# HiLab-git/FPL-plus

Measured on AMD Instinct MI355X. Metric: 3D volumes/sec (train step, 80x160x160), higher is better.
Workload: dtype bf16; 1 GPU; UNet3D-DSBN 32-base-ch bf16 (fp32 master weights), per-GPU batch 2x1x80x160x160 synthetic VS crops, DiceLoss + Adam, domain alternating per step; global_batch=2, parallelism=dp1, step=zero_grad+forward+loss+backward+allreduce+adam

## Files before the change

fpl-plus_amd/csrc/common.h:

```cpp
#pragma once
#include <hip/hip_runtime.h>
#include <math.h>
#include <stdint.h>
#include <stdio.h>
#include <stdarg.h>
#include <string.h>
#include "../../include/fplx.h"

typedef __bf16 bf16_t;

#define FPLX_WAVE 64

inline char* fplx_err_buf() {
  static thread_local char buf[512];
  return buf;
}
inline int fplx_fail(int code, const char* fmt, ...) {
  va_list ap;
  va_start(ap, fmt);
  vsnprintf(fplx_err_buf(), 512, fmt, ap);
  va_end(ap);
  return code;
}
inline int fplx_check_launch(const char* what) {
  hipError_t e = hipGetLastError();
  if (e != hipSuccess) return fplx_fail(FPLX_E_HIP, "%s: %s", what, hipGetErrorString(e));
  return FPLX_OK;
}
#define FPLX_REQUIRE(cond, code, ...) \
  do {                                 \
    if (!(cond)) return fplx_fail(code, __VA_ARGS__); \
  } while (0)

template <typename T> struct Act;
template <> struct Act<float> {
  static __device__ __forceinline__ float ld(const float* p) { return *p; }
  static __device__ __forceinline__ void st(float* p, float v) { *p = v; }
};
template <> struct Act<bf16_t> {
  static __device__ __forceinline__ float ld(const bf16_t* p) { return (float)*p; }
  static __device__ __forceinline__ void st(bf16_t* p, float v) { *p = (bf16_t)v; }
};

__device__ __forceinline__ float ld_dt(const void* p, int64_t i, int dt) {
  return dt == FPLX_F32 ? ((const float*)p)[i] : (float)((const bf16_t*)p)[i];
}
__device__ __forceinline__ void st_dt(void* p, int64_t i, int dt, float v) {
  if (dt == FPLX_F32) ((float*)p)[i] = v;
  else ((bf16_t*)p)[i] = (bf16_t)v;
}

__device__ __forceinline__ float wave_sum(float v) {
#pragma unroll
  for (int o = 32; o > 0; o >>= 1) v += __shfl_xor(v, o, 64);
  return v;
}
__device__ __forceinline__ double wave_sum_d(double v) {
#pragma unroll
  for (int o = 32; o > 0; o >>= 1) v += __shfl_xor(v, o, 64);
  return v;
}

#ifdef __HIPCC__
struct FplxAdamConst { float step_size, b1, b2, eps, wd, inv_sqrt_bc2, gscale, omb1, omb2; };
__device__ __forceinline__ void fplx_adam_elem(float& pi, float g, float& mi, float& vi, const FplxAdamConst& c) {
  const float gi = fmaf(c.wd, pi, g * c.gscale);
  mi = fmaf(c.b1, mi, c.omb1 * gi);
  vi = fmaf(c.b2, vi, (c.omb2 * gi) * gi);
  const float denom = fmaf(sqrtf(vi), c.inv_sqrt_bc2, c.eps);
  pi = fmaf(-c.step_size, mi / denom, pi);
}
struct FplxOptimConst { float lr, wd, gscale, k0, k1, k2, k3, k4; int first; };
__device__ __forceinline__ float fplx_optim_grad(float pi, float g, const FplxOptimConst& c) {
  return fmaf(c.wd, pi, g * c.gscale);
}
template <bool MOM>
__device__ __forceinline__ void fplx_sgd_elem(float& pi, float g, float& buf, const FplxOptimConst& c) {
  const float gi = fplx_optim_grad(pi, g, c);
  if (MOM) {
    buf = fmaf(c.k0, buf, gi);
    pi = fmaf(-c.lr, buf, pi);
  } else {
    pi = fmaf(-c.lr, gi, pi);
  }
}
__device__ __forceinline__ void fplx_adadelta_elem(float& pi, float g, float& sq, float& acc, const FplxOptimConst& c) {
  const float gi = fplx_optim_grad(pi, g, c);
  sq = fmaf(c.k0, sq, (c.k1 * gi) * gi);
  const float stdv = sqrtf(sq + c.k2);
  const float ratio = sqrtf(acc + c.k2) / stdv;
  const float delta = ratio * gi;
  acc = fmaf(c.k0, acc, (c.k1 * delta) * delta);
  pi = fmaf(-c.lr, delta, pi);
}
__device__ __forceinline__ void fplx_adagrad_elem(float& pi, float g, float& sum, const FplxOptimConst& c) {
  const float gi = fplx_optim_grad(pi, g, c);
  sum = fmaf(gi, gi, sum);
  const float stdv = sqrtf(sum) + c.k2;
  pi = fmaf(-c.lr, gi / stdv, pi);
}
__device__ __forceinline__ void fplx_adamax_elem(float& pi, float g, float& mi, float& ui, const FplxOptimConst& c) {
  const float gi = fplx_optim_grad(pi, g, c);
  mi = fmaf(c.k0, mi, c.k1 * gi);
  const float decayed = c.k3 * ui;
  ui = fmaxf(decayed, fabsf(gi) + c.k2);
  pi = fmaf(-c.lr, mi / ui, pi);
}
__device__ __forceinline__ void fplx_asgd_elem(float& pi, float g, float& ax, const FplxOptimConst& c) {
  const float gi = fplx_optim_grad(pi, g, c);
  const float decayed = pi * c.k0;
  pi = fmaf(-c.lr, gi, decayed);
  const float d = pi - ax;
  ax = c.k3 == 1.f ? pi : fmaf(d, c.k3, ax);
}
template <bool MOM>
__device__ __forceinline__ void fplx_rmsprop_elem(float& pi, float g, float& sq, float& buf, const FplxOptimConst& c) {
  const float gi = fplx_optim_grad(pi, g, c);
  sq = fmaf(c.k0, sq, (c.k1 * gi) * gi);
  const float avg = sqrtf(sq) + c.k2;
  if (MOM) {
    buf = fmaf(c.k3, buf, gi / avg);
    pi = fmaf(-c.lr, buf, pi);
  } else {
    pi = fmaf(-c.lr, gi / avg, pi);
  }
}
__device__ __forceinline__ void fplx_rprop_elem(float& pi, float g, float& prev, float& ss, const FplxOptimConst& c) {
  float gi = g * c.gscale;
  if (c.first) { prev = 0.f; ss = c.lr; }
  const float s = gi * prev;
  const float f = s > 0.f ? c.k1 : (s < 0.f ? c.k0 : 1.f);
  const float scaled = ss * f;
  ss = fminf(fmaxf(scaled, c.k3), c.k4);
  if (s < 0.f) gi = 0.f;
  const float sg = gi > 0.f ? 1.f : (gi < 0.f ? -1.f : 0.f);
  pi = fmaf(-sg, ss, pi);
  prev = gi;
}
template <int KIND, int NS>
__device__ __forceinline__ void fplx_optim_elem(float& pi, float g, float& s0, float& s1, const FplxOptimConst& c) {
  if constexpr (KIND == FPLX_OPT_SGD) fplx_sgd_elem<NS == 1>(pi, g, s0, c);
  else if constexpr (KIND == FPLX_OPT_ADADELTA) fplx_adadelta_elem(pi, g, s0, s1, c);
  else if constexpr (KIND == FPLX_OPT_ADAGRAD) fplx_adagrad_elem(pi, g, s0, c);
  else if constexpr (KIND == FPLX_OPT_ADAMAX) fplx_adamax_elem(pi, g, s0, s1, c);
  else if constexpr (KIND == FPLX_OPT_ASGD) fplx_asgd_elem(pi, g, s0, c);
  else if constexpr (KIND == FPLX_OPT_RMSPROP) fplx_rmsprop_elem<NS == 2>(pi, g, s0, s1, c);
  else fplx_rprop_elem(pi, g, s0, s1, c);
}
#define FPLX_OPTIM_DISPATCH(kind, ns, X)                                       \
  switch ((kind) * 4 + (ns)) {                                                 \
    case FPLX_OPT_SGD * 4 + 0: X(FPLX_OPT_SGD, 0); break;                      \
    case FPLX_OPT_SGD * 4 + 1: X(FPLX_OPT_SGD, 1); break;                      \
    case FPLX_OPT_ADADELTA * 4 + 2: X(FPLX_OPT_ADADELTA, 2); break;            \
    case FPLX_OPT_ADAGRAD * 4 + 1: X(FPLX_OPT_ADAGRAD, 1); break;              \
    case FPLX_OPT_ADAMAX * 4 + 2: X(FPLX_OPT_ADAMAX, 2); break;                \
    case FPLX_OPT_ASGD * 4 + 1: X(FPLX_OPT_ASGD, 1); break;                    \
    case FPLX_OPT_RMSPROP * 4 + 1: X(FPLX_OPT_RMSPROP, 1); break;              \
    case FPLX_OPT_RMSPROP * 4 + 2: X(FPLX_OPT_RMSPROP, 2); break;              \
    default: X(FPLX_OPT_RPROP, 2); break;                                      \
  }
static inline int fplx_optim_consts(const char* who, int kind, const float* hp, int nhp, int step, float gscale, const void* s0,
                                    const void* s1, FplxOptimConst* c, int* ns) {
  static const int want[FPLX_OPT_COUNT] = {3, 4, 4, 5, 4, 5, 5};
  FPLX_REQUIRE(kind >= 0 && kind < FPLX_OPT_COUNT, FPLX_E_BADSHAPE, "%s: unknown optimiser kind %d (0..%d)", who, kind,
               FPLX_OPT_COUNT - 1);
  FPLX_REQUIRE(hp, FPLX_E_NULL, "%s: null hyper-parameter array", who);
  FPLX_REQUIRE(nhp == want[kind], FPLX_E_BADSHAPE, "%s: kind %d takes %d hyper-parameters, got %d", who, kind, want[kind], nhp);
  FPLX_REQUIRE(step >= 1, FPLX_E_BADSHAPE, "%s: step=%d (1-based)", who, step);
  *c = {hp[0], 0.f, gscale, 0.f, 0.f, 0.f, 0.f, 0.f, step == 1};
  int need = 2;
  switch (kind) {
    case FPLX_OPT_SGD:
      c->k0 = hp[1]; c->wd = hp[2];
      need = hp[1] != 0.f ? 1 : 0;
      break;
    case FPLX_OPT_ADADELTA:
      c->k0 = hp[1]; c->k1 = (float)(1.0 - (double)hp[1]); c->k2 = hp[2]; c->wd = hp[3];
      break;
    case FPLX_OPT_ADAGRAD:
      c->lr = (float)((double)hp[0] / (1.0 + (double)(step - 1) * (double)hp[1])); c->k2 = hp[2]; c->wd = hp[3];
      need = 1;
      break;
    case FPLX_OPT_ADAMAX:
      c->lr = (float)((double)hp[0] / (1.0 - pow((double)hp[1], step)));
      c->k0 = hp[1]; c->k1 = (float)(1.0 - (double)hp[1]); c->k3 = hp[2]; c->k2 = hp[3]; c->wd = hp[4];
      break;
    case FPLX_OPT_ASGD:
      c->k0 = (float)(1.0 - (double)hp[2] * (double)hp[0]); c->k3 = hp[1]; c->wd = hp[3];
      need = 1;
      break;
    case FPLX_OPT_RMSPROP:
      c->k0 = hp[1]; c->k1 = (float)(1.0 - (double)hp[1]); c->k2 = hp[2]; c->k3 = hp[3]; c->wd = hp[4];
      need = hp[3] > 0.f ? 2 : 1;
      break;
    default:
      c->k0 = hp[1]; c->k1 = hp[2]; c->k3 = hp[3]; c->k4 = hp[4];
      break;
  }
  FPLX_REQUIRE((need < 1 || s0) && (need < 2 || s1), FPLX_E_NULL, "%s: kind %d needs %d state buffer(s) here", who, kind, need);
  *ns = need;
  return FPLX_OK;
}
struct FplxBlock { int x, y, z; };
__device__ __forceinline__ FplxBlock fplx_xcd_block(int on) {
  FplxBlock b = {(int)blockIdx.x, (int)blockIdx.y, (int)blockIdx.z};
  if (!on) return b;
  const unsigned gx = gridDim.x, gy = gridDim.y, gz = gridDim.z, t = gx * gy * gz;
  const unsigned l = (blockIdx.z * gy + blockIdx.y) * gx + blockIdx.x;
  const unsigned xcd = l & 7u, q = t >> 3, r = t & 7u;
  const unsigned lp = xcd * q + (xcd < r ? xcd : r) + (l >> 3);
  const unsigned per = gy * gz, xq = lp / per, rem = lp - xq * per;
  b.x = __builtin_amdgcn_readfirstlane((int)xq);
  b.z = __builtin_amdgcn_readfirstlane((int)(rem / gy));
  b.y = __builtin_amdgcn_readfirstlane((int)(rem % gy));
  return b;
}
struct FplxTileRange { int64_t first, end, step; };
__device__ __forceinline__ FplxTileRange fplx_xcd_tiles(int64_t ntiles, int on) {
  FplxTileRange t = {(int64_t)blockIdx.x, ntiles, (int64_t)gridDim.x};
  if (!on || gridDim.x < 16) return t;
  const unsigned c = blockIdx.x & 7u, xcd = (blockIdx.y * gridDim.x + blockIdx.x) & 7u;
  const int64_t q = ntiles >> 3, r = ntiles & 7;
  const int64_t start = xcd * q + ((int64_t)xcd < r ? xcd : r);
  t.first = start + (blockIdx.x >> 3);
  t.end = start + q + ((int64_t)xcd < r ? 1 : 0);
  t.step = (gridDim.x - c + 7u) >> 3;
  return t;
}
template <typename... P, typename... A>
inline void fplx_launch(void (*kernel)(P...), dim3 grid, dim3 block, size_t lds, hipStream_t st, A... args) {
  if (lds) (void)hipFuncSetAttribute((const void*)kernel, hipFuncAttributeMaxDynamicSharedMemorySize, (int)lds);
  kernel<<<grid, block, lds, st>>>(args...);
}
#endif
#define FPLX_KNOB_LIST(X)                                                                                              \
  X(XCD, "xcd", 1)                                                    \
  X(BRICK, "brick", 1)                                    \
  X(BRICK_FILL, "brick_fill", 192)           \
  X(BRICK_GEO, "brick_geo", -1)                    \
  X(BRICK_KSPLIT, "brick_ksplit", 0)                                             \
  X(EDGE_BLOCKS, "edge_blocks", 1024)                             \
  X(STEM_ROWS, "stem_rows", 1)                                              \
  X(OUTCONV_T, "outconv_t", 1)                                 \
  X(OUTCONV_DGRAD_MFMA, "outconv_dgrad_mfma", 1)                                                                       \
  X(OUTCONV_FWD_ROWS, "outconv_fwd_rows", 1)  \
  X(OUTCONV_DGRAD_ROWS, "outconv_dgrad_rows", 1)  \
  X(PACK_TILED, "pack_tiled", 1)                                                                                       \
  X(PACK_MULTI, "pack_multi", 1)                                                                                       \
  X(MARCH, "march", 1)                               \
  X(MARCH64_FW, "march64_fw", 0)                                \
  X(MARCH_DS, "march_ds", 0)                                       \
  X(MARCH128, "march128", 1)                                                                                           \
  X(MARCH64_LW, "march64_lw", 1)            \
  X(MARCH32_V2, "march32_v2", 4)              \
  X(WG_COT_MINVOX, "wg_cot_minvox", 0)                                                                                 \
  X(WG_TW, "wg_tw", 0)                                                                                                 \
  X(WG_CIT, "wg_cit", 2)                                                                                               \
  X(WG_COT, "wg_cot", 2)                                                                                               \
  X(WG_DS, "wg_ds", 0)                                                                                                 \
  X(WG_VOX, "wg_vox", 1)                              \
  X(WG_ROLL, "wg_roll", 1)                     \
  X(WG_ROLL_GEO, "wg_roll_geo", 0)          \
  X(WG_ROLL_M16, "wg_roll_m16", 1)                 \
  X(WG_ROLL_MB, "wg_roll_mb", 1)            \
  X(WG_ROLL_CUS, "wg_roll_cus", 256)                                \
  X(WG_ROLL_OVH, "wg_roll_ovh", 9)                     \
  X(WG_ROLL_MINVOX, "wg_roll_minvox", 0)                                                   \
  X(WG_ROLL2D, "wg_roll2d", 1)              \
  X(WG_ROLL2D_OVH, "wg_roll2d_ovh", 3)      \
  X(WG_REDUCE_ROWS, "wg_reduce_rows", 8)    \
  X(WG_VOX_LW, "wg_vox_lw", 1)              \
  X(WG_VOX_CUS, "wg_vox_cus", 128)          \
  X(WG_VOX_MAXV, "wg_vox_maxv", 10000)         \
  X(STREAM_MIN_W, "stream_min_w", 64)                                                                                  \
  X(TILE_MT, "tile_mt", 0)                                                                                             \
  X(TILE_NT, "tile_nt", 0)                                                                                             \
  X(TILE_KS, "tile_ks", 0)                                                                                             \
  X(MID_TILE, "mid_tile", 1)                                                                                           \
  X(DECONV_ROWS, "deconv_rows", 1)                                                                                     \
  X(DECONV_DGRAD_ROWS, "deconv_dgrad_rows", 1)   \
  X(ROWS_SMALL_DIV, "rows_small_div", 16)   \
  X(EW_GROUP, "ew_group", 1)                                                                                           \
  X(POOL_COL, "pool_col", 1)                         \
  X(EW_INFLIGHT, "ew_inflight", 2)          \
  X(EW_INFLIGHT_REDUCE, "ew_inflight_reduce", 2)
enum FplxKnobId {
#define FPLX_KNOB_ENUM(id, key, def) FPLX_K_##id,
  FPLX_KNOB_LIST(FPLX_KNOB_ENUM)
#undef FPLX_KNOB_ENUM
  FPLX_K_COUNT
};
extern "C" __attribute__((visibility("hidden"))) int64_t fplx_knob_values[FPLX_K_COUNT];
static inline int64_t fplx_knob(int id) { return __atomic_load_n(&fplx_knob_values[id], __ATOMIC_RELAXED); }
static inline int fplx_xcd_on() { return (int)fplx_knob(FPLX_K_XCD); }

static inline int fplx_rows_for(int64_t voxels) {
  constexpr int cap = 512;
  const int div = voxels <= 32768 ? (int)fplx_knob(FPLX_K_ROWS_SMALL_DIV) : 64;
  int64_t r = (voxels + div - 1) / div;
  if (r > cap) r = cap;
  if (r < 1) r = 1;
  return (int)r;
}
```

fpl-plus_amd/csrc/conv_mfma.hip:

```cpp
#include "internal.h"
#include "gfx950.h"
#include <stdlib.h>

namespace {

constexpr int DIRECT_THREADS = 256;

template <int MT, int NTL, int MODE>
__global__ void __launch_bounds__(DIRECT_THREADS)
conv_fwd_direct(const bf16_t* __restrict__ x, int64_t ldx, const bf16_t* __restrict__ wp,
                const float* __restrict__ bias, bf16_t* __restrict__ y, int64_t ldy, int N, int D, int H, int W,
                int Cin, int Cout, float* __restrict__ stats, float* __restrict__ partial = nullptr) {
  const int lane = threadIdx.x & 63, wave = threadIdx.x >> 6;
  const int r = lane & 31, kh8 = (lane >> 5) * 8;
  const int64_t V = (int64_t)N * D * H * W;
  const int64_t m0 = ((int64_t)blockIdx.x * 4 + wave) * (MT * 32);
  const int n0 = blockIdx.y * (NTL * 32);

  int vn[MT], vd[MT], vh[MT], vw[MT];
  bool vok[MT];
#pragma unroll
  for (int t = 0; t < MT; ++t) {
    int64_t v = m0 + t * 32 + r;
    vok[t] = v < V;
// ... 1929 lines not shown
  bool fits;
  StreamCfg stream;
  DirectCfg direct;
};

static FwdPlan fwd_plan(int n, int d, int h, int w, int cin, int cout, int mid) {
  FwdPlan p = {};
  p.kernel = FPLX_KERNEL_GENERIC; p.geo = -1; p.ksplit = 1; p.tap_cnt = 27;
  if (cin % 16 != 0 || cout % 32 != 0) return p;
  const int64_t V = (int64_t)n * d * h * w;
  p.fits = V < ((int64_t)1 << 31);
  auto split = [&](int rows) {
    p.stats_rows = p.ksplit > 1 ? splitk_fin_blocks(V) : rows;
    p.ws_bytes = p.ksplit > 1 ? (size_t)p.ksplit * V * cout * sizeof(float) : 0;
  };
  auto brick = [&]() {
    int bricks;
    fplx_brick_plan(n, d, h, w, cin, cout, &p.geo, &p.ksplit, &bricks);
    p.kernel = FPLX_KERNEL_BRICK;
    split(bricks);
  };
  if (!mid && fplx_brick_first(n, d, h, w, cin, cout)) { brick(); return p; }
  if (fplx_march_ok(n, d, h, w, cin, cout)) {
    p.kernel = FPLX_KERNEL_MARCH;
    p.geo = fplx_march_variant(n, d, h, w, cin, cout);
    p.stats_rows = fplx_march_rows(n, d, h, w, cin, cout);
    return p;
  }
  if (stream_ok(d, h, w, cin, cout)) {
    p.kernel = FPLX_KERNEL_STREAM;
    p.stream = stream_cfg(n, d, h, w, cout);
    p.stats_rows = p.stream.nblk;
    return p;
  }
  if (!mid && fplx_brick_ok(n, d, h, w, cin, cout)) { brick(); return p; }
  if (mid && fplx_knob(FPLX_K_MID_TILE) != 0 && cin % 32 == 0 && cout % 64 == 0) { p.tap_lo = 9; p.tap_cnt = 9; }
  p.direct = direct_cfg(V, cin, cout, p.tap_cnt);
  p.kernel = p.direct.tile_nt ? FPLX_KERNEL_TILE : FPLX_KERNEL_DIRECT;
  p.ksplit = p.direct.ksplit;
  split((int)p.direct.mblocks);
  return p;
}

extern "C" int fplx_mfma_conv3d_plan(int n, int d, int h, int w, int cin, int cout, int mid, int* kernel, int* geo, int* ksplit) {
  const FwdPlan p = fwd_plan(n, d, h, w, cin, cout, mid);
  const bool ok = p.kernel != FPLX_KERNEL_GENERIC && p.fits;
  *kernel = ok ? p.kernel : FPLX_KERNEL_GENERIC; *geo = ok ? p.geo : -1; *ksplit = ok ? p.ksplit : 1;
  return ok;
}
extern "C" int fplx_mfma_conv3d_stats_rows(int n, int d, int h, int w, int cin, int cout, int mid) {
  return fwd_plan(n, d, h, w, cin, cout, mid).stats_rows;
}
extern "C" size_t fplx_mfma_conv3d_fwd_ws_bytes(int n, int d, int h, int w, int cin, int cout, int mid) {
  return fwd_plan(n, d, h, w, cin, cout, mid).ws_bytes;
}

static int mfma_fwd_impl(const void* x, int64_t ldx, const void* wp, const float* bias, void* y, int64_t ldy, int n, int d,
                         int h, int w, int cin, int cout, float* stats, void* ws, size_t ws_bytes, int mid,
                         hipStream_t st, const float* slope = nullptr) {
  if (!mfma_applicable(ldx, ldy, cin, cout, x, y, wp)) return 0;
  const FwdPlan p = fwd_plan(n, d, h, w, cin, cout, mid);
  if (!p.fits) return 0;
  const int64_t V = (int64_t)n * d * h * w;
  const int ks = p.ksplit;
  if (ks > 1 && (!ws || ws_bytes < p.ws_bytes))
    return fplx_fail(FPLX_E_WORKSPACE, "mfma_conv3d_fwd: split-K needs %zu workspace bytes (fplx_conv3d_fwd_ws_bytes)", p.ws_bytes);
  float* partial = ks > 1 ? (float*)ws : nullptr;
  switch (p.kernel) {
    case FPLX_KERNEL_BRICK: {
      const int rb = fplx_brick_conv3d_fwd_act(x, ldx, wp, bias, y, ldy, n, d, h, w, cin, cout, stats, (float*)ws, p.geo, ks,
                                               st, slope, nullptr, 0);
      if (rb == 1 && ks > 1) {
        splitk_finish_k<<<splitk_fin_blocks(V), 256, 0, st>>>((const float*)ws, ks, V, cout, bias, (bf16_t*)y, ldy, stats, slope);
        const int rf = fplx_check_launch("brick_splitk_finish");
        if (rf < 0) return rf;
      }
      return rb;
    }
    case FPLX_KERNEL_MARCH:
      return fplx_march_conv3d_fwd_act(x, ldx, wp, bias, y, ldy, n, d, h, w, cin, cout, stats, st, nullptr, nullptr, mid, slope, 0);
    case FPLX_KERNEL_STREAM: {
      if (slope) return 0;
      const StreamCfg& sc = p.stream;
      const auto k = cin == 32 ? conv_fwd_stream<32> : conv_fwd_stream<64>;
      fplx_launch(k, dim3(sc.nblk, cout / 32), 256, cin == 32 ? StreamGeo<32>::LDS : StreamGeo<64>::LDS, st, (const bf16_t*)x, ldx,
                  (const bf16_t*)wp, bias, (bf16_t*)y, ldy, n, d, h, w, cout, stats, sc.tilesH, sc.tilesW, sc.dsegs, sc.dlen);
      int rc0 = fplx_check_launch("mfma_conv3d_fwd_stream");
      return rc0 < 0 ? rc0 : 1;
    }
    case FPLX_KERNEL_TILE: {
      if (slope && ks <= 1) return 0;
      const DirectCfg& c = p.direct;
      const bool k64 = cin % 64 == 0;
      const int kc = (c.tile_mt == 256 || k64) ? 64 : 32;
      const auto k = c.tile_mt == 256 ? (c.tile_nt == 128 ? conv_fwd_tile<128, 64, 256> : conv_fwd_tile<64, 64, 256>)
                     : c.tile_nt == 128 ? (k64 ? conv_fwd_tile<128, 64, 128> : conv_fwd_tile<128, 32, 128>)
                                        : (k64 ? conv_fwd_tile<64, 64, 128> : conv_fwd_tile<64, 32, 128>);
      fplx_launch(k, dim3((unsigned)c.mblocks, cout / c.tile_nt, ks), c.tile_mt * 2, (size_t)2 * (c.tile_mt + c.tile_nt) * kc * 2, st,
                  (const bf16_t*)x, ldx, (const bf16_t*)wp, bias, (bf16_t*)y, ldy, n, d, h, w, cin, cout, stats, partial, p.tap_lo,
                  p.tap_cnt, fplx_xcd_on());
      if (ks > 1) splitk_finish_k<<<c.fin_blocks, 256, 0, st>>>(partial, ks, V, cout, bias, (bf16_t*)y, ldy, stats, slope);
      int rct = fplx_check_launch("mfma_conv3d_fwd_tile");
      return rct < 0 ? rct : 1;
    }
    case FPLX_KERNEL_DIRECT: {
      if (slope && ks <= 1) return 0;
      const DirectCfg& c = p.direct;
      const auto k = c.ntl == 2 ? conv_fwd_direct<2, 2, 0> : conv_fwd_direct<4, 1, 0>;
      fplx_launch(k, dim3((unsigned)c.mblocks, cout / (c.ntl * 32), ks), DIRECT_THREADS, 0, st, (const bf16_t*)x, ldx,
                  (const bf16_t*)wp, bias, (bf16_t*)y, ldy, n, d, h, w, cin, cout, stats, partial);
      if (ks > 1) splitk_finish_k<<<c.fin_blocks, 256, 0, st>>>(partial, ks, V, cout, bias, (bf16_t*)y, ldy, stats, slope);
      int rc = fplx_check_launch("mfma_conv3d_fwd");
      return rc < 0 ? rc : 1;
    }
    default: return 0;
  }
}

extern "C" int fplx_mfma_conv3d_fwd(const void* x, int64_t ldx, const void* wp, const float* bias, void* y, int64_t ldy,
                                    int n, int d, int h, int w, int cin, int cout, float* stats, void* ws,
                                    size_t ws_bytes, int mid, hipStream_t st) {
  return mfma_fwd_impl(x, ldx, wp, bias, y, ldy, n, d, h, w, cin, cout, stats, ws, ws_bytes, mid, st);
}

static inline bool act_sample_fits(int d, int h, int w, int cin) {
  return (int64_t)d * h * w * (2 * cin) * 2 < ((int64_t)1 << 30);
}
extern "C" int fplx_mfma_conv3d_act_ok(int n, int d, int h, int w, int cin, int cout, int mid) {
  if (!act_sample_fits(d, h, w, cin)) return 0;
  const FwdPlan p = fwd_plan(n, d, h, w, cin, cout, mid);
  if (!p.fits) return 0;
  return p.kernel == FPLX_KERNEL_BRICK || p.kernel == FPLX_KERNEL_MARCH ||
         ((p.kernel == FPLX_KERNEL_TILE || p.kernel == FPLX_KERNEL_DIRECT) && p.ksplit > 1);
}
static inline bool act_cat2_plan(const FwdPlan& p, int d, int h, int w, int cin, int mid) {
  return !mid && cin % 64 == 0 && act_sample_fits(d, h, w, cin) && p.fits && p.kernel == FPLX_KERNEL_BRICK && p.ksplit == 1;
}
extern "C" int fplx_mfma_conv3d_act_cat2_ok(int n, int d, int h, int w, int cin, int cout, int mid) {
  return act_cat2_plan(fwd_plan(n, d, h, w, cin, cout, mid), d, h, w, cin, mid);
}
extern "C" int fplx_mfma_conv3d_fwd_act_cat2(const void* x0, const void* x1, int64_t ldx, const void* wp, const float* bias,
                                             const float* slope, void* y, int64_t ldy, int n, int d, int h, int w, int cin,
                                             int cout, int nmod0, hipStream_t st) {
  const FwdPlan p = fwd_plan(n, d, h, w, cin, cout, 0);
  if (!act_cat2_plan(p, d, h, w, cin, 0) || !mfma_applicable(ldx, ldy, cin, cout, x0, y, wp)) return 0;
  return fplx_brick_conv3d_fwd_act(x0, ldx, wp, bias, y, ldy, n, d, h, w, cin, cout, nullptr, nullptr, p.geo, p.ksplit, st, slope, x1, nmod0);
}
extern "C" int fplx_mfma_conv3d_fwd_act(const void* x, int64_t ldx, const void* wp, const float* bias, const float* slope, void* y,
                                        int64_t ldy, int n, int d, int h, int w, int cin, int cout, void* ws, size_t ws_bytes,
                                        int mid, hipStream_t st) {
  return mfma_fwd_impl(x, ldx, wp, bias, y, ldy, n, d, h, w, cin, cout, nullptr, ws, ws_bytes, mid, st, slope);
}

enum { WG_VOX, WG_ROLL, WG_STREAM };
struct WgradPlan { int kernel; size_t ws_bytes; VoxCfg vox; WgCfg stream; };

static WgradPlan wgrad_plan(int n, int d, int h, int w, int cin, int cout, int mid, int splitx) {
  WgradPlan p = {};
  if (!splitx && !mid) {
    p.vox = vox_cfg(n, d, h, w, cin, cout);
    if (p.vox.ok) { p.kernel = WG_VOX; p.ws_bytes = p.vox.ws; return p; }
  }
  if (fplx_wgroll_ok(n, d, h, w, cin, cout, mid, splitx)) {
    p.kernel = WG_ROLL;
    p.ws_bytes = fplx_wgroll_ws_bytes(n, d, h, w, cin, cout);
    return p;
  }
  p.kernel = WG_STREAM;
  p.stream = wg_cfg(n, d, h, w, cin, cout);
  p.ws_bytes = p.stream.ws;
  return p;
}

extern "C" int fplx_wgrad_reduce_launch(const float* part, int nblk, int npairs, int cin, int cout, float* dw, int mid,
                                        hipStream_t st) {
  wgrad_finish(part, nblk, npairs, cin, cout, dw, mid, st);
  return fplx_check_launch("wgrad_stream_reduce");
}

extern "C" int fplx_mfma_conv3d_wgrad_cit(int n, int d, int h, int w, int cin, int cout) {
  if (cin % 32 != 0 || cout % 32 != 0) return 0;
  return wg_cfg(n, d, h, w, cin, cout).cit;
}

extern "C" size_t fplx_mfma_conv3d_wgrad_ws_bytes(int n, int d, int h, int w, int cin, int cout) {
  if (cin % 32 != 0 || cout % 32 != 0) return 0;
  size_t m = wg_cfg(n, d, h, w, cin, cout).ws;
  const VoxCfg v = vox_cfg(n, d, h, w, cin, cout);
  if (v.ok && v.ws > m) m = v.ws;
  if (fplx_wgroll_ok(n, d, h, w, cin, cout, 0, 0)) { const size_t r = fplx_wgroll_ws_bytes(n, d, h, w, cin, cout); if (r > m) m = r; }
  return m;
}

extern "C" int fplx_mfma_conv3d_wgrad(const void* x, int64_t ldx, const void* dy, int64_t ldy, float* dw, int n, int d,
                                      int h, int w, int cin, int cout, void* ws, size_t ws_bytes, hipStream_t st,
                                      const void* x1, int mid) {
  if (cin % 32 != 0 || cout % 32 != 0 || ldx % 8 != 0 || ldy % 8 != 0 || ((uintptr_t)x % 16) || ((uintptr_t)dy % 16))
    return 0;
  WgradPlan p = wgrad_plan(n, d, h, w, cin, cout, mid, x1 != nullptr);
  if (p.kernel == WG_VOX) {
    const VoxCfg& v = p.vox;
    if (ws_bytes < v.ws) return fplx_fail(FPLX_E_WORKSPACE, "mfma_conv3d_wgrad: workspace %zu < %zu", ws_bytes, v.ws);
    const int lwk = (int)fplx_knob(FPLX_K_WG_VOX_LW);
    const bool lw = (lwk == 2 || (lwk == 1 && v.g.V <= 2048)) && v.cot == 1 && (int64_t)v.g.V * ldx * 2 < ((int64_t)1 << 31) &&
                    (int64_t)v.g.V * ldy * 2 < ((int64_t)1 << 31);
    const auto k = lw ? conv_wgrad_vox_lw : v.cot == 2 ? conv_wgrad_vox<2> : conv_wgrad_vox<1>;
    fplx_launch(k, dim3(v.g.S, v.npairs / v.cot), lw ? 512 : 256, v.lds, st, (const bf16_t*)x, ldx, (const bf16_t*)dy, ldy,
                (float*)ws, cin, cout, v.g, fplx_xcd_on());
    wgrad_finish((const float*)ws, v.g.S, v.npairs, cin, cout, dw, 0, st);
    int rcv = fplx_check_launch("mfma_conv3d_wgrad_vox");
    return rcv < 0 ? rcv : 1;
  }
  if (p.kernel == WG_ROLL) {
    const int rr = fplx_wgroll_conv3d_wgrad(x, ldx, dy, ldy, dw, n, d, h, w, cin, cout, ws, ws_bytes, st, x1, mid);
    if (rr != 0) return rr;
    p.stream = wg_cfg(n, d, h, w, cin, cout);
  }
  const WgCfg& c = p.stream;
  if (x1 && (c.cit != 2 || cin != 64 || ((uintptr_t)x1 % 16))) return 0;
  if (ws_bytes < c.ws) return fplx_fail(FPLX_E_WORKSPACE, "mfma_conv3d_wgrad: workspace %zu < %zu", ws_bytes, c.ws);
#define WG_KERNEL(TW_, CIT_, COT_) (mid ? conv_wgrad_stream<TW_, CIT_, COT_, true> : conv_wgrad_stream<TW_, CIT_, COT_, false>)
  const int tw = c.tw == 32 ? 32 : 16, cot = c.cot == 2 ? 2 : 1, cit = (cot == 1 && c.cit == 2) ? 2 : 1;
  const auto k = tw == 32 ? (cot == 2 ? WG_KERNEL(32, 1, 2) : cit == 2 ? WG_KERNEL(32, 2, 1) : WG_KERNEL(32, 1, 1))
                          : (cot == 2 ? WG_KERNEL(16, 1, 2) : cit == 2 ? WG_KERNEL(16, 2, 1) : WG_KERNEL(16, 1, 1));
#undef WG_KERNEL
  fplx_launch(k, dim3(c.nblk, c.npairs / (c.cit * c.cot)), 256, (size_t)(3 * cit * (WG_TH + 2) * (tw + 2) + cot * WG_TH * tw) * 64, st,
              (const bf16_t*)x, ldx, (const bf16_t*)dy, ldy, (float*)ws, n, d, h, w, cin, cout, c.tilesH, c.tilesW, c.dsegs, c.dlen,
              (const bf16_t*)x1, fplx_xcd_on());
  wgrad_finish((const float*)ws, c.nblk, c.npairs, cin, cout, dw, mid, st);
  int rc = fplx_check_launch("mfma_conv3d_wgrad");
  return rc < 0 ? rc : 1;
}

extern "C" int fplx_mfma_deconv2_fwd(const void* x, int64_t ldx, const void* wf, const float* bias, void* y, int64_t ldy,
                                     int n, int d, int h, int w, int cin, int cout, int sd, hipStream_t st) {
  if (cin % 32 != 0 || cout % 32 != 0 || ldx % 8 != 0 || ((uintptr_t)x % 16) || ((uintptr_t)wf % 16)) return 0;
  const int64_t V = (int64_t)n * d * h * w;
  if (V >= ((int64_t)1 << 31)) return 0;
  const int vec_ok = ldy % 8 == 0 && ((uintptr_t)y % 16) == 0;
  {
    const int krows = (int)fplx_knob(FPLX_K_DECONV_ROWS);
    const int ks = cin / 16, ntc = cout / 32;
    if (krows && sd == 2 && vec_ok && V >= 32 * 1024 && ((ks == 4 && ntc == 1) || (ks == 8 && ntc == 2) || (ks == 8 && ntc == 1) ||
                                                         (ks == 4 && ntc == 2))) {
      const int64_t nt = (V + 31) / 32;
      const unsigned nb = (unsigned)(nt < 1024 ? nt : 1024);
      auto launch = [&](auto kernel) {
        fplx_launch(kernel, nb, 256, 0, st, (const bf16_t*)x, ldx, (const bf16_t*)wf, bias, (bf16_t*)y, ldy, n, d, h, w, fplx_xcd_on());
      };
      if (ks == 4 && ntc == 1) launch(deconv_fwd_rows<4, 1>);
      else if (ks == 8 && ntc == 2) launch(deconv_fwd_rows<8, 2>);
      else if (ks == 8 && ntc == 1) launch(deconv_fwd_rows<8, 1>);
      else launch(deconv_fwd_rows<4, 2>);
      int rc = fplx_check_launch("mfma_deconv2_fwd_rows");
      return rc < 0 ? rc : 1;
    }
  }
  dim3 grid((unsigned)((V + 127) / 128), cout / 32, sd);
  deconv_fwd_mfma<<<grid, DIRECT_THREADS, 0, st>>>((const bf16_t*)x, ldx, (const bf16_t*)wf, bias, (bf16_t*)y, ldy, n, d,
                                                   h, w, cin, cout, sd, vec_ok, fplx_xcd_on());
  int rc = fplx_check_launch("mfma_deconv2_fwd");
  return rc < 0 ? rc : 1;
}

extern "C" int fplx_mfma_deconv2_dgrad(const void* dy, int64_t ldy, const void* wb, void* dx, int64_t ldx, int n, int d,
                                       int h, int w, int cin, int cout, int sd, hipStream_t st) {
  if (cout % 16 != 0 || cin % 32 != 0 || ldy % 8 != 0 || ((uintptr_t)dy % 16) || ((uintptr_t)wb % 16)) return 0;
  const int64_t V = (int64_t)n * d * h * w;
  if (V * 8 >= ((int64_t)1 << 31)) return 0;
  if (sd == 2 && fplx_knob(FPLX_K_DECONV_DGRAD_ROWS) && V >= 16 * 1024 && ldx % 8 == 0 && ((uintptr_t)dx % 16) == 0 &&
      ((cout == 32 && cin == 64) || (cout == 64 && cin == 128))) {
    const int mb = cin == 64 ? 64 : 32;
    const int segsW = (w + mb - 1) / mb;
    const int64_t nseg = (int64_t)n * d * h * segsW;
    const unsigned nb = (unsigned)(nseg < 512 ? nseg : 512);
    if (cout == 32)
      deconv_dgrad_rows<1, 2><<<nb, 256, 0, st>>>((const bf16_t*)dy, ldy, (const bf16_t*)wb, (bf16_t*)dx, ldx, n, d, h, w, segsW, nseg, fplx_xcd_on());
    else
      deconv_dgrad_rows<2, 4><<<nb, 256, 0, st>>>((const bf16_t*)dy, ldy, (const bf16_t*)wb, (bf16_t*)dx, ldx, n, d, h, w, segsW, nseg, fplx_xcd_on());
    int rcr = fplx_check_launch("mfma_deconv2_dgrad_rows");
    return rcr < 0 ? rcr : 1;
  }
  if (sd == 2 && fplx_knob(FPLX_K_DECONV_DGRAD_ROWS) && ((V + 127) / 128) * (cin / 64) < 128 && cin % 64 == 0 && cout % 16 == 0 &&
      ldx % 8 == 0 && ((uintptr_t)dx % 16) == 0) {
    dim3 gs((unsigned)((V + 31) / 32), cin / 64);
    deconv_dgrad_small<<<gs, 256, 0, st>>>((const bf16_t*)dy, ldy, (const bf16_t*)wb, (bf16_t*)dx, ldx, n, d, h, w, cout, cin);
    int rcs = fplx_check_launch("mfma_deconv2_dgrad_small");
    return rcs < 0 ? rcs : 1;
  }
  const bool wide = cin % 64 == 0;
  const dim3 grid = wide ? dim3((unsigned)((V + 255) / 256), cin / 64) : dim3((unsigned)((V + 511) / 512), cin / 32);
  const bool deep = wide && (int64_t)grid.x * grid.y < 192;
  const auto k = deep ? (sd == 2 ? conv_fwd_direct<1, 2, 1> : conv_fwd_direct<1, 2, 2>)
                 : wide ? (sd == 2 ? conv_fwd_direct<2, 2, 1> : conv_fwd_direct<2, 2, 2>)
                        : (sd == 2 ? conv_fwd_direct<4, 1, 1> : conv_fwd_direct<4, 1, 2>);
  fplx_launch(k, deep ? dim3((unsigned)((V + 127) / 128), cin / 64) : grid, DIRECT_THREADS, 0, st, (const bf16_t*)dy, ldy,
              (const bf16_t*)wb, nullptr, (bf16_t*)dx, ldx, n, d, h, w, cout, cin, nullptr, nullptr);
  int rc = fplx_check_launch("mfma_deconv2_dgrad");
  return rc < 0 ? rc : 1;
}

extern "C" size_t fplx_mfma_deconv2_wgrad_ws_bytes(int n, int d, int h, int w, int cin, int cout) {
  if (cin % 32 != 0 || cout % 32 != 0) return 0;
  return dw_cfg(n, d, h, w, cin, cout).ws;
}

extern "C" int fplx_mfma_deconv2_wgrad(const void* x, int64_t ldx, const void* dy, int64_t ldy, float* dw, float* db,
                                       int n, int d, int h, int w, int cin, int cout, void* ws, size_t ws_bytes,
                                       int sd, hipStream_t st) {
  if (cin % 32 != 0 || cout % 32 != 0 || ldx % 8 != 0 || ldy % 8 != 0 || ((uintptr_t)x % 16) || ((uintptr_t)dy % 16))
    return 0;
  const DwCfg c = dw_cfg(n, d, h, w, cin, cout);
  if (ws_bytes < c.ws) return fplx_fail(FPLX_E_WORKSPACE, "mfma_deconv2_wgrad: workspace %zu < %zu", ws_bytes, c.ws);
  const size_t lds = (size_t)(c.cit + 8) * 128 * 64;
  float* bpart = db ? (float*)((char*)ws + (size_t)c.nblk * c.npairs * 8 * c.cit * 1024 * sizeof(float)) : nullptr;
  auto launch = [&](auto kernel) {
    fplx_launch(kernel, dim3(c.nblk, c.npairs), 256, lds, st, (const bf16_t*)x, ldx, (const bf16_t*)dy, ldy, (float*)ws, bpart, n, d,
                h, w, cin, cout, sd);
  };
  if (c.cit == 4) launch(deconv_wgrad_mfma<4>);
  else if (c.cit == 2) launch(deconv_wgrad_mfma<2>);
  else launch(deconv_wgrad_mfma<1>);
  const int64_t total = (int64_t)c.npairs * 8 * c.cit * 1024;
  if (db) deconv_bias_reduce<<<cout, 64, 0, st>>>(bpart, c.nblk, cout, db);
  deconv_wgrad_reduce<<<(unsigned)((total + 63) / 64), 256, 0, st>>>((const float*)ws, c.nblk, c.npairs, c.cit, cin, cout, dw,
                                                                      4 * sd);
  int rc = fplx_check_launch("mfma_deconv2_wgrad");
  return rc < 0 ? rc : 1;
}
```

fpl-plus_amd/csrc/internal.h:

```cpp
#pragma once
#include "common.h"

extern "C" {

int fplx_march_ok(int n, int d, int h, int w, int cin, int cout);
int fplx_march_rows(int n, int d, int h, int w, int cin, int cout);
int fplx_march_variant(int n, int d, int h, int w, int cin, int cout);
int fplx_march_conv3d_fwd(const void* x, int64_t ldx, const void* wp, const float* bias, void* y, int64_t ldy, int n, int d,
                          int h, int w, int cin, int cout, float* stats, hipStream_t st, const void* x1, void* y1, int twod);
int fplx_march_conv3d_fwd_act(const void* x, int64_t ldx, const void* wp, const float* bias, void* y, int64_t ldy, int n,
                              int d, int h, int w, int cin, int cout, float* stats, hipStream_t st, const void* x1, void* y1,
                              int twod, const float* slope, int nmod0);

int fplx_brick_ok(int n, int d, int h, int w, int cin, int cout);
int fplx_brick_first(int n, int d, int h, int w, int cin, int cout);
int fplx_brick_plan(int n, int d, int h, int w, int cin, int cout, int* geo, int* ksplit, int* bricks);
int fplx_brick_conv3d_fwd_act(const void* x, int64_t ldx, const void* wp, const float* bias, void* y, int64_t ldy, int n,
                              int d, int h, int w, int cin, int cout, float* stats, float* partial, int geo, int ksplit,
                              hipStream_t st, const float* slope, const void* x1, int nmod0);

int fplx_wgroll_ok(int n, int d, int h, int w, int cin, int cout, int mid, int splitx);
size_t fplx_wgroll_ws_bytes(int n, int d, int h, int w, int cin, int cout);
int fplx_wgroll_conv3d_wgrad(const void* x, int64_t ldx, const void* dy, int64_t ldy, float* dw, int n, int d, int h, int w,
                             int cin, int cout, void* ws, size_t ws_bytes, hipStream_t st, const void* x1, int mid);

int fplx_mfma_conv3d_plan(int n, int d, int h, int w, int cin, int cout, int mid, int* kernel, int* geo, int* ksplit);
int fplx_mfma_conv3d_stats_rows(int n, int d, int h, int w, int cin, int cout, int mid);
size_t fplx_mfma_conv3d_fwd_ws_bytes(int n, int d, int h, int w, int cin, int cout, int mid);
int fplx_mfma_conv3d_fwd(const void* x, int64_t ldx, const void* wp, const float* bias, void* y, int64_t ldy, int n, int d,
                         int h, int w, int cin, int cout, float* stats, void* ws, size_t ws_bytes, int mid, hipStream_t st);
int fplx_mfma_conv3d_act_ok(int n, int d, int h, int w, int cin, int cout, int mid);
int fplx_mfma_conv3d_act_cat2_ok(int n, int d, int h, int w, int cin, int cout, int mid);
int fplx_mfma_conv3d_fwd_act(const void* x, int64_t ldx, const void* wp, const float* bias, const float* slope, void* y,
                             int64_t ldy, int n, int d, int h, int w, int cin, int cout, void* ws, size_t ws_bytes, int mid,
                             hipStream_t st);
int fplx_mfma_conv3d_fwd_act_cat2(const void* x0, const void* x1, int64_t ldx, const void* wp, const float* bias,
                                  const float* slope, void* y, int64_t ldy, int n, int d, int h, int w, int cin, int cout,
                                  int nmod0, hipStream_t st);
int fplx_mfma_conv3d_wgrad_cit(int n, int d, int h, int w, int cin, int cout);
size_t fplx_mfma_conv3d_wgrad_ws_bytes(int n, int d, int h, int w, int cin, int cout);
int fplx_mfma_conv3d_wgrad(const void* x, int64_t ldx, const void* dy, int64_t ldy, float* dw, int n, int d, int h, int w,
                           int cin, int cout, void* ws, size_t ws_bytes, hipStream_t st, const void* x1, int mid);
int fplx_wgrad_reduce_launch(const float* part, int nblk, int npairs, int cin, int cout, float* dw, int mid, hipStream_t st);
int fplx_mfma_deconv2_fwd(const void* x, int64_t ldx, const void* wf, const float* bias, void* y, int64_t ldy, int n, int d,
                          int h, int w, int cin, int cout, int sd, hipStream_t st);
int fplx_mfma_deconv2_dgrad(const void* dy, int64_t ldy, const void* wb, void* dx, int64_t ldx, int n, int d, int h, int w,
                            int cin, int cout, int sd, hipStream_t st);
size_t fplx_mfma_deconv2_wgrad_ws_bytes(int n, int d, int h, int w, int cin, int cout);
int fplx_mfma_deconv2_wgrad(const void* x, int64_t ldx, const void* dy, int64_t ldy, float* dw, float* db, int n, int d,
                            int h, int w, int cin, int cout, void* ws, size_t ws_bytes, int sd, hipStream_t st);

int fplx_edge_stem_rows(int n, int d, int h, int w, int cin, int cout);
int fplx_edge_stem_fwd(const float* x, const void* wf, const float* bias, void* y, int64_t ldy, int n, int d, int h, int w,
                       int cin, int cout, float* stats, hipStream_t st);
size_t fplx_edge_stem_wgrad_ws_bytes(int n, int d, int h, int w, int cin, int cout);
int fplx_edge_stem_wgrad(const float* x, const void* dy, int64_t ldy, float* dw, int n, int d, int h, int w, int cin,
                         int cout, void* ws, hipStream_t st);
int fplx_edge_stem_wgrad_bn(const float* x, const void* dy, int64_t ldy, float* dw, int n, int d, int h, int w, int cin,
                            int cout, void* ws, hipStream_t st, const void* y, int64_t ldyy, const float* mean,
                            const float* rstd, const float* scale, const float* shift, const float* slope, const float* coef);
int fplx_edge_outconv_fwd(const void* x, int64_t ldx, const float* wf, const float* bias, float* out, int n, int d, int h,
                          int w, int cin, int ncls, hipStream_t st);
int fplx_edge_outconv_dgrad(const float* dl, const void* wb, void* dx, int64_t ldx, int n, int d, int h, int w, int c0,
                            int ncls, hipStream_t st);
size_t fplx_edge_outconv_wgrad_ws_bytes(int n, int d, int h, int w, int c0, int ncls);
int fplx_edge_outconv_wgrad(const void* x, int64_t ldx, const float* dl, float* dw, int n, int d, int h, int w, int c0,
                            int ncls, void* ws, hipStream_t st);
int fplx_edge_outconv_bn_ok(int n, int d, int h, int w, int c0, int ncls);
int fplx_edge_outconv_bn_rows(int n, int d, int h, int w, int ncls);
int fplx_edge_outconv_fwd_bn(const void* y, int64_t ldy, const float* scale, const float* shift, const float* slope, void* a,
                             int64_t lda, const float* wf, const float* bias, float* out, int n, int d, int h, int w, int c0,
                             int ncls, hipStream_t st);
int fplx_edge_outconv_dgrad_bn(int mode, const float* dl, const void* wb, const void* y, int64_t ldy, const float* mean,
                               const float* rstd, const float* scale, const float* shift, const float* slope,
                               const float* coef, float* part, void* dy, int64_t lddy, int n, int d, int h, int w, int c0,
                               int ncls, hipStream_t st);
size_t fplx_edge_outconv_wgrad_bn_ws_bytes(int n, int d, int h, int w, int c0, int ncls);
int fplx_edge_outconv_wgrad_bn(const void* y, int64_t ldy, const float* scale, const float* shift, const float* slope,
                               const float* dl, float* dw, float* db, int n, int d, int h, int w, int c0, int ncls, void* ws,
                               hipStream_t st);

}
```

Before: 254.3 volumes/s.

## Add double-buffered pipelined MFMA kernel for stride-2 deconv weight gradient

Adds a new deconv wgrad path for stride 2, on by default. Blocks walk voxel chunks grid-stride and prefetch the next chunk into registers while MFMAs consume the current LDS slot. Block count comes from a small cost model that balances streaming time against partial-sum reduction traffic. A new finish kernel reduces the partials and bias in one launch. The cost is more workspace and a second code path with its own correctness risks.

```diff
diff --git a/fpl-plus_amd/csrc/common.h b/fpl-plus_amd/csrc/common.h
--- a/fpl-plus_amd/csrc/common.h
+++ b/fpl-plus_amd/csrc/common.h
@@ -279,6 +279,8 @@
   X(MID_TILE, "mid_tile", 1)                                                                                           \
   X(DECONV_ROWS, "deconv_rows", 1)                                                                                     \
   X(DECONV_DGRAD_ROWS, "deconv_dgrad_rows", 1)   \
+  X(DECONV_WGRAD_PIPE, "deconv_wgrad_pipe", 1)   \
+  X(DECONV_WGRAD_NBLK, "deconv_wgrad_nblk", 0)   \
   X(ROWS_SMALL_DIV, "rows_small_div", 16)   \
   X(EW_GROUP, "ew_group", 1)                                                                                           \
   X(POOL_COL, "pool_col", 1)                         \
diff --git a/fpl-plus_amd/csrc/conv_mfma.hip b/fpl-plus_amd/csrc/conv_mfma.hip
--- a/fpl-plus_amd/csrc/conv_mfma.hip
+++ b/fpl-plus_amd/csrc/conv_mfma.hip
@@ -2255,7 +2255,8 @@
 
 extern "C" size_t fplx_mfma_deconv2_wgrad_ws_bytes(int n, int d, int h, int w, int cin, int cout) {
   if (cin % 32 != 0 || cout % 32 != 0) return 0;
-  return dw_cfg(n, d, h, w, cin, cout).ws;
+  const size_t a = dw_cfg(n, d, h, w, cin, cout).ws, b = fplx_deconv_wgrad_pipe_ws_bytes(n, d, h, w, cin, cout);
+  return a > b ? a : b;
 }
 
 extern "C" int fplx_mfma_deconv2_wgrad(const void* x, int64_t ldx, const void* dy, int64_t ldy, float* dw, float* db,
@@ -2263,6 +2264,10 @@
                                        int sd, hipStream_t st) {
   if (cin % 32 != 0 || cout % 32 != 0 || ldx % 8 != 0 || ldy % 8 != 0 || ((uintptr_t)x % 16) || ((uintptr_t)dy % 16))
     return 0;
+  if (sd == 2 && fplx_knob(FPLX_K_DECONV_WGRAD_PIPE)) {
+    const int rp = fplx_deconv_wgrad_pipe(x, ldx, dy, ldy, dw, db, n, d, h, w, cin, cout, ws, ws_bytes, st);
+    if (rp != 0) return rp;
+  }
   const DwCfg c = dw_cfg(n, d, h, w, cin, cout);
   if (ws_bytes < c.ws) return fplx_fail(FPLX_E_WORKSPACE, "mfma_deconv2_wgrad: workspace %zu < %zu", ws_bytes, c.ws);
   const size_t lds = (size_t)(c.cit + 8) * 128 * 64;
diff --git a/fpl-plus_amd/csrc/deconv_wgrad_pipe.hip b/fpl-plus_amd/csrc/deconv_wgrad_pipe.hip
--- /dev/null
+++ b/fpl-plus_amd/csrc/deconv_wgrad_pipe.hip
@@ -0,0 +1,250 @@
+#include "gfx950.h"
+#include "internal.h"
+
+namespace {
+
+constexpr int KV = 64;
+
+template <int CIT, int TW>
+__global__ void __launch_bounds__(256, 2)
+deconv_wgrad_pipe(const bf16_t* __restrict__ x, int64_t ldx, const bf16_t* __restrict__ dy, int64_t ldy,
+                  float* __restrict__ part, float* __restrict__ bpart, int D, int H, int W, unsigned V, int chunks, int Cin,
+                  int Cout) {
+  constexpr int TPB = 4 * TW, NTG = 8 / TPB;
+  constexpr int SLOT = (CIT + TPB) * KV * 64;
+  extern __shared__ __attribute__((aligned(16))) char smem[];
+  const int tid = threadIdx.x, lane = tid & 63;
+  const int wave = __builtin_amdgcn_readfirstlane(tid >> 6);
+  const int ncig = Cin / (32 * CIT);
+  const int tg = blockIdx.y % NTG, pair = blockIdx.y / NTG;
+  const int cot = pair / ncig, cig = pair % ncig;
+  const int g = lane >> 4, q = (lane & 15) >> 2, p = lane & 3;
+  const int lane_off = (8 * (g >> 1) + q) * 64 + (16 * (g & 1) + 4 * p) * 2;
+  const int c16 = tid & 3, vox = tid >> 2;
+  const bool want_bias = bpart != nullptr && cig == 0;
+  const bf16_t* xcol = x + (cig * CIT) * 32 + c16 * 8;
+  const bf16_t* dycol = dy + cot * 32 + c16 * 8;
+  float bsum[8];
+#pragma unroll
+  for (int j = 0; j < 8; ++j) bsum[j] = 0.f;
+  f32x16 acc[TW][CIT];
+#pragma unroll
+  for (int t = 0; t < TW; ++t)
+#pragma unroll
+    for (int c = 0; c < CIT; ++c)
+#pragma unroll
+      for (int i = 0; i < 16; ++i) acc[t][c][i] = 0.f;
+
+  uint4 xv[CIT], gv[TPB];
+  auto fetch = [&](int ch) {
+    const unsigned vv = (unsigned)ch * KV + vox;
+#pragma unroll
+    for (int c = 0; c < CIT; ++c) xv[c] = make_uint4(0, 0, 0, 0);
+#pragma unroll
+    for (int tl = 0; tl < TPB; ++tl) gv[tl] = make_uint4(0, 0, 0, 0);
+    if (vv < V) {
+      const bf16_t* xr = xcol + (int64_t)vv * ldx;
+#pragma unroll
+      for (int c = 0; c < CIT; ++c) xv[c] = *reinterpret_cast<const uint4*>(xr + c * 32);
+      unsigned r = vv;
+      const unsigned w0 = r % (unsigned)W; r /= (unsigned)W;
+      const unsigned h0 = r % (unsigned)H; r /= (unsigned)H;
+      const unsigned d0 = r % (unsigned)D; r /= (unsigned)D;
+      const unsigned ob = ((r * 2u * D + 2u * d0) * 2u * H + 2u * h0) * 2u * W + 2u * w0;
+#pragma unroll
+      for (int tl = 0; tl < TPB; ++tl) {
+        const int tap = tg * TPB + tl;
+        const unsigned ov = ob + ((unsigned)(tap >> 2) * 2u * H + ((tap >> 1) & 1)) * 2u * W + (tap & 1);
+        gv[tl] = *reinterpret_cast<const uint4*>(dycol + (int64_t)ov * ldy);
+      }
+    }
+  };
+  auto stage = [&](char* slot) {
+#pragma unroll
+    for (int c = 0; c < CIT; ++c) *reinterpret_cast<uint4*>(slot + (c * KV + vox) * 64 + c16 * 16) = xv[c];
+#pragma unroll
+    for (int tl = 0; tl < TPB; ++tl) {
+      *reinterpret_cast<uint4*>(slot + ((CIT + tl) * KV + vox) * 64 + c16 * 16) = gv[tl];
+      if (want_bias) {
+        const bf16x8 b8 = *reinterpret_cast<const bf16x8*>(&gv[tl]);
+#pragma unroll
+        for (int j = 0; j < 8; ++j) bsum[j] += (float)b8[j];
+      }
+    }
+  };
+
+  int ch = blockIdx.x;
+  fetch(ch);
+  stage(smem);
+  lds_barrier();
+  for (int it = 0;; ++it) {
+    const int next = ch + (int)gridDim.x;
+    const bool more = next < chunks;
+    if (more) fetch(next);
+    const char* xs = smem + (it & 1) * SLOT;
+    const char* dys = xs + CIT * KV * 64;
+#pragma unroll
+    for (int ks = 0; ks < KV / 16; ++ks) {
+      bf16x8 bfr[TW];
+#pragma unroll
+      for (int t = 0; t < TW; ++t) bfr[t] = tr_frag(dys + ((wave * TW + t) * KV + ks * 16) * 64 + lane_off);
+#pragma unroll
+      for (int c = 0; c < CIT; ++c) {
+        const bf16x8 afr = tr_frag(xs + (c * KV + ks * 16) * 64 + lane_off);
+#pragma unroll
+        for (int t = 0; t < TW; ++t) acc[t][c] = __builtin_amdgcn_mfma_f32_32x32x16_bf16(afr, bfr[t], acc[t][c], 0, 0, 0);
+      }
+    }
+    if (!more) break;
+    stage(smem + ((it + 1) & 1) * SLOT);
+    lds_barrier();
+    ch = next;
+  }
+
+  float* out = part + ((int64_t)blockIdx.x * (gridDim.y / NTG) + pair) * (8 * CIT * 1024);
+#pragma unroll
+  for (int t = 0; t < TW; ++t)
+#pragma unroll
+    for (int c = 0; c < CIT; ++c) {
+      float* tile = out + ((tg * TPB + wave * TW + t) * CIT + c) * 1024;
+#pragma unroll
+      for (int j = 0; j < 4; ++j) {
+        f32x4 v4;
+#pragma unroll
+        for (int k = 0; k < 4; ++k) v4[k] = acc[t][c][4 * j + k];
+        *reinterpret_cast<f32x4*>(tile + (j * 64 + lane) * 4) = v4;
+      }
+    }
+  if (want_bias) {
+    lds_barrier();
+    float* red = reinterpret_cast<float*>(smem);
+#pragma unroll
+    for (int j = 0; j < 8; ++j) red[tid * 8 + j] = bsum[j];
+    lds_barrier();
+    if (tid < 32) {
+      const int cc = tid >> 3, j = tid & 7;
+      float t = 0.f;
+      for (int k = 0; k < 64; ++k) t += red[(k * 4 + cc) * 8 + j];
+      bpart[((int64_t)blockIdx.x * NTG + tg) * Cout + cot * 32 + tid] = t;
+    }
+  }
+}
+
+__global__ void __launch_bounds__(256)
+deconv_wgrad_pipe_finish(const float* __restrict__ part, const float* __restrict__ bpart, int nblk, int brows, int ncolblk,
+                         int cpb, int cit, int Cin, int Cout, float* __restrict__ dw, float* __restrict__ db) {
+  __shared__ f32x4 red[256];
+  const int tid = threadIdx.x;
+  if ((int)blockIdx.x >= ncolblk) {
+    float* redf = reinterpret_cast<float*>(red);
+    const int c = ((int)blockIdx.x - ncolblk) * 16 + (tid & 15), s = tid >> 4;
+    float t = 0.f;
+    for (int r = s; r < brows; r += 16) t += bpart[(int64_t)r * Cout + c];
+    redf[tid] = t;
+    __syncthreads();
+    if (tid < 16) {
+      float a = 0.f;
+#pragma unroll
+      for (int k = 0; k < 16; ++k) a += redf[k * 16 + tid];
+      db[c] = a;
+    }
+    return;
+  }
+  const int S = 256 / cpb, s = tid / cpb, cl = tid % cpb;
+  const int64_t ncols = (int64_t)Cin * Cout * 2;
+  const int64_t col = (int64_t)blockIdx.x * cpb + cl;
+  const f32x4* src = reinterpret_cast<const f32x4*>(part) + col;
+  f32x4 a = {0.f, 0.f, 0.f, 0.f};
+  int b = s;
+  for (; b + 3 * S < nblk; b += 4 * S) {
+    const f32x4 v0 = src[(int64_t)b * ncols], v1 = src[(int64_t)(b + S) * ncols], v2 = src[(int64_t)(b + 2 * S) * ncols],
+                v3 = src[(int64_t)(b + 3 * S) * ncols];
+    a += v0; a += v1; a += v2; a += v3;
+  }
+  for (; b < nblk; b += S) a += src[(int64_t)b * ncols];
+  if (S > 1) {
+    red[tid] = a;
+    __syncthreads();
+    if (s != 0) return;
+    a = red[cl];
+    for (int k = 1; k < S; ++k) a += red[k * cpb + cl];
+  }
+  const int tile = (int)(col >> 8), j = (int)(col >> 6) & 3, ln = (int)col & 63;
+  const int c = tile % cit, tap = (tile / cit) & 7, pair = tile / (8 * cit);
+  const int ncig = Cin / (32 * cit);
+  const int co = (pair / ncig) * 32 + (ln & 31), ci = ((pair % ncig) * cit + c) * 32 + 8 * j + 4 * (ln >> 5);
+#pragma unroll
+  for (int k = 0; k < 4; ++k) dw[((int64_t)(ci + k) * Cout + co) * 8 + tap] = a[k];
+}
+
+struct PipePlan { int cit, ntg, npairs, chunks, nblk_max, nblk; size_t tile_bytes, ws; };
+
+inline PipePlan pipe_plan(int n, int d, int h, int w, int cin, int cout) {
+  PipePlan p;
+  p.cit = (cin % 128 == 0) ? 4 : (cin % 64 == 0 ? 2 : 1);
+  const int64_t V = (int64_t)n * d * h * w;
+  const int chunks128 = (int)((V + 127) / 128);
+  p.ntg = (p.cit == 4 && chunks128 >= 2) ? 2 : 1;
+  p.npairs = (cin / (32 * p.cit)) * (cout / 32);
+  p.chunks = (int)((V + KV - 1) / KV);
+  int cap = 512 / (p.npairs * p.ntg), lim = chunks128 / p.ntg;
+  if (cap > lim) cap = lim;
+  if (cap < 1) cap = 1;
+  p.nblk_max = cap;
+  p.tile_bytes = (size_t)cin * cout * 8 * sizeof(float);
+  const double T_CHUNK = 3.0;
+  const double stream = (double)V * (cin + 8 * cout) * 2 / 5e6;
+  double best = 0;
+  p.nblk = 1;
+  for (int nb = 1; nb <= cap; ++nb) {
+    const double walk = (double)((p.chunks + nb - 1) / nb) * T_CHUNK;
+    const double t = (stream > walk ? stream : walk) + (double)nb * p.tile_bytes * 2 / 4e6;
+    if (nb == 1 || t < best) { best = t; p.nblk = nb; }
+  }
+  if (p.nblk >= 16) p.nblk &= ~7;
+  const int64_t force = fplx_knob(FPLX_K_DECONV_WGRAD_NBLK);
+  if (force > 0) p.nblk = force < cap ? (int)force : cap;
+  p.ws = (size_t)p.nblk_max * (p.tile_bytes + (size_t)p.ntg * cout * sizeof(float));
+  return p;
+}
+
+inline bool pipe_shape_ok(int n, int d, int h, int w, int cin, int cout) {
+  return cin % 32 == 0 && cout % 32 == 0 && (int64_t)n * d * h * w * 8 < ((int64_t)1 << 31) &&
+         (int64_t)(cin / 32) * (cout / 32) <= 512;
+}
+
+}
+
+extern "C" size_t fplx_deconv_wgrad_pipe_ws_bytes(int n, int d, int h, int w, int cin, int cout) {
+  if (!pipe_shape_ok(n, d, h, w, cin, cout)) return 0;
+  return pipe_plan(n, d, h, w, cin, cout).ws;
+}
+
+extern "C" int fplx_deconv_wgrad_pipe(const void* x, int64_t ldx, const void* dy, int64_t ldy, float* dw, float* db, int n,
+                                      int d, int h, int w, int cin, int cout, void* ws, size_t ws_bytes, hipStream_t st) {
+  if (!pipe_shape_ok(n, d, h, w, cin, cout) || ldx % 8 != 0 || ldy % 8 != 0 || ((uintptr_t)x % 16) || ((uintptr_t)dy % 16) ||
+      ((uintptr_t)ws % 16))
+    return 0;
+  const PipePlan p = pipe_plan(n, d, h, w, cin, cout);
+  if (ws_bytes < p.ws) return fplx_fail(FPLX_E_WORKSPACE, "deconv_wgrad_pipe: workspace %zu < %zu", ws_bytes, p.ws);
+  float* part = (float*)ws;
+  float* bpart = db ? (float*)((char*)ws + (size_t)p.nblk * p.tile_bytes) : nullptr;
+  const unsigned V = (unsigned)((int64_t)n * d * h * w);
+  const dim3 grid(p.nblk, p.npairs * p.ntg);
+  auto launch = [&](auto kernel, int tpb) {
+    fplx_launch(kernel, grid, 256, (size_t)2 * (p.cit + tpb) * KV * 64, st, (const bf16_t*)x, ldx, (const bf16_t*)dy, ldy, part,
+                bpart, d, h, w, V, p.chunks, cin, cout);
+  };
+  if (p.cit == 4 && p.ntg == 2) launch(deconv_wgrad_pipe<4, 1>, 4);
+  else if (p.cit == 4) launch(deconv_wgrad_pipe<4, 2>, 8);
+  else if (p.cit == 2) launch(deconv_wgrad_pipe<2, 2>, 8);
+  else launch(deconv_wgrad_pipe<1, 2>, 8);
+  const int64_t ncols = (int64_t)cin * cout * 2;
+  int S = 1;
+  while (S < 16 && ncols * S < 65536 && 2 * S <= p.nblk) S *= 2;
+  const int cpb = 256 / S, ncolblk = (int)(ncols / cpb);
+  deconv_wgrad_pipe_finish<<<ncolblk + (db ? cout / 16 : 0), 256, 0, st>>>(part, bpart, p.nblk, p.nblk * p.ntg, ncolblk, cpb, p.cit,
+                                                                          cin, cout, dw, db);
+  const int rc = fplx_check_launch("deconv_wgrad_pipe");
+  return rc < 0 ? rc : 1;
+}
diff --git a/fpl-plus_amd/csrc/internal.h b/fpl-plus_amd/csrc/internal.h
--- a/fpl-plus_amd/csrc/internal.h
+++ b/fpl-plus_amd/csrc/internal.h
@@ -50,6 +50,10 @@
 int fplx_mfma_deconv2_wgrad(const void* x, int64_t ldx, const void* dy, int64_t ldy, float* dw, float* db, int n, int d,
                             int h, int w, int cin, int cout, void* ws, size_t ws_bytes, int sd, hipStream_t st);
 
+size_t fplx_deconv_wgrad_pipe_ws_bytes(int n, int d, int h, int w, int cin, int cout);
+int fplx_deconv_wgrad_pipe(const void* x, int64_t ldx, const void* dy, int64_t ldy, float* dw, float* db, int n, int d, int h,
+                           int w, int cin, int cout, void* ws, size_t ws_bytes, hipStream_t st);
+
 int fplx_edge_stem_rows(int n, int d, int h, int w, int cin, int cout);
 int fplx_edge_stem_fwd(const float* x, const void* wf, const float* bias, void* y, int64_t ldy, int n, int d, int h, int w,
                        int cin, int cout, float* stats, hipStream_t st);
```

Result: no change. 255.5 volumes/s, median of 6 (+0.5%).
